# JuanTarrio/rebvo

Measured on NVIDIA H100. Metric: frames/sec @752x480 EuRoC replay (synthetic stand-in), detect+track+map; pose ATE vs reference in `parity`, higher is better.
Workload: dtype f32 scale space/detector + f64 tracker/EKF

## Files before the change

rebvo_b200/csrc/capi.cu:

```cuda
#include <math.h>
#include <stdlib.h>
#include <new>

#include "common.cuh"
#include "tracker.cuh"

int rb_detect_upload_pinv(rb_ctx *c);

static void box_plan_one(double sigma, int box_n, int *box_d, double *sigma_r) {
    const double wideal = sqrt(12 * sigma * sigma / box_n + 1);
    int wl = (int)wideal;
    const int tmp = wl / 2;
    if (tmp * 2 == wl) wl--;
    const int m = (int)round((3 * box_n + 4 * box_n * wl + box_n * wl * wl - 12 * sigma * sigma) / (4 + 4 * wl));
    int i = 0;
    for (; i < m && i < box_n; i++) box_d[i] = wl;
    for (; i < box_n; i++) box_d[i] = wl + 2;
    *sigma_r = sqrt((m * wl * wl + (box_n - m) * (wl + 2.0) * (wl + 2.0) - box_n) / 12.0);
}

static void plane_fit_pinv(double pinv[3][25]) {
    const int ws = 2;
    double Phi[25][3];
    int k = 0;
// ... 119 lines not shown
    kl.n_m0[i] = k.n_m0;
    kl.p_id[i] = k.p_id;
    kl.n_id[i] = k.n_id;
    kl.pack[2 * i] = make_float4(k.m_m[0], k.m_m[1], k.c_p[0], k.c_p[1]);
    kl.pack[2 * i + 1] = make_float4(k.u_m[0], k.u_m[1], k.n_m, 0.f);
}

__global__ void k_fill_int(int *p, int v, size_t n) {
    size_t i = (size_t)blockIdx.x * blockDim.x + threadIdx.x;
    if (i < n) p[i] = v;
}

extern "C" int rb_ctx_create(rb_ctx **out, int device, const rb_camera *cam, double sigma0, double ksigma,
                             int kl_capacity) {
    if (!out || !cam) return RB_ERR_ARG;
    *out = nullptr;
    int ndev = 0;
    if (cudaGetDeviceCount(&ndev) != cudaSuccess || ndev <= 0 || device >= ndev) return RB_ERR_NO_DEVICE;
    if (cam->w % 4 || cam->w < 32 || cam->h < 32 || kl_capacity < 1) return RB_ERR_ARG;
    rb_ctx *c = new (std::nothrow) rb_ctx;
    if (!c) return RB_ERR_ARG;
    memset(c, 0, sizeof(*c));
    c->mtx = new (std::nothrow) std::recursive_mutex;
    if (!c->mtx) {
        delete c;
        return RB_ERR_ARG;
    }
    c->device = device;
    c->cam = *cam;
    c->w = cam->w;
    c->h = cam->h;
    c->N = cam->w * cam->h;
    c->ppx = cam->ppx;
    c->ppy = cam->ppy;
    c->zfm = (double)((cam->zfx + cam->zfy) / 2);
    c->sigma0 = sigma0;
    c->ksigma = ksigma;
    c->kcap = kl_capacity;
    {
        const char *ds = getenv("REBVO_B200_DOG_SUB");
        c->dog_sub = ds ? atoi(ds) : 0;
        if (c->dog_sub < 0) c->dog_sub = 0;
        const char *pd = getenv("REBVO_B200_PDL");
        c->pdl = !(pd && atoi(pd) == 0);
        const char *mp = getenv("REBVO_B200_MIN_PERSIST");
        c->min_persist = !(mp && atoi(mp) == 0);
        const char *mc = getenv("REBVO_B200_MIN_CLUSTER");
        c->min_cluster = !(mc && atoi(mc) == 0);
        const char *rs = getenv("REBVO_B200_ROWSCAN");
        c->rowscan_mode = rs ? atoi(rs) : 2;
        c->mu_xchg = !(getenv("REBVO_B200_MU_XCHG") && atoi(getenv("REBVO_B200_MU_XCHG")) == 0);
        c->row_ns = getenv("REBVO_B200_ROW_NS") ? atoi(getenv("REBVO_B200_ROW_NS")) : 0;
        c->colscan_mode = getenv("REBVO_B200_COLSCAN") ? atoi(getenv("REBVO_B200_COLSCAN")) : 0;
    }
    box_plan_one(sigma0, 3, c->plan.d[0], &c->plan.sigma_r[0]);
    box_plan_one(c->plan.sigma_r[0] * ksigma, 3, c->plan.d[1], &c->plan.sigma_r[1]);
    plane_fit_pinv(c->pinv);
    int r = RB_OK;
    auto fail = [&](int code) {
        *out = c;
        return code;
    };
#define CK(call)                                                                                  \
    do {                                                                                          \
        cudaError_t e__ = (call);                                                                 \
        if (e__ != cudaSuccess) {                                                                 \
            snprintf(c->err, sizeof(c->err), "%s:%d %s: %s", __FILE__, __LINE__, #call,           \
                     cudaGetErrorString(e__));                                                    \
            return fail(RB_ERR_CUDA);                                                             \
        }                                                                                         \
    } while (0)
    CK(cudaSetDevice(device));
    cudaDeviceProp prop;
    CK(cudaGetDeviceProperties(&prop, device));
    c->sm_count = prop.multiProcessorCount;
    rb_minimizer_cluster_setup(c);
    if ((r = rb_dog_device_setup(c))) return fail(r);
    {
        int lo = 0, hi = 0;
        cudaDeviceGetStreamPriorityRange(&lo, &hi);
        const char *pe = getenv("REBVO_B200_PRIO");
        CK(cudaStreamCreateWithPriority(&c->stream, cudaStreamNonBlocking, (pe && atoi(pe) == 0) ? lo : hi));
    }
    c->nseg = c->h * rb_div_up(c->w, 32);
    CK(cudaMalloc(&c->seg_cnt, sizeof(int) * c->nseg));
    CK(cudaMalloc(&c->cand, sizeof(float4) * (size_t)c->N));
    c->red_cap = 1024;
    CK(cudaMalloc(&c->red_part, sizeof(double) * 32 * c->red_cap));
    CK(cudaMalloc(&c->ticket, sizeof(unsigned int) * 16));
    CK(cudaMemset(c->ticket, 0, sizeof(unsigned int) * 16));
    CK(cudaMallocHost(&c->pinned, 1 << 16));
    CK(cudaMalloc(&c->dev_small, 1 << 16));
    CK(cudaMemset(c->dev_small, 0, 1 << 16));
    {
        const int mm_init[2] = {-1, 0x7f7fffff};
        CK(cudaMemcpy((char *)c->dev_small + RB_DS_REEST, mm_init, sizeof(mm_init), cudaMemcpyHostToDevice));
    }
    if ((r = rb_detect_upload_pinv(c))) return fail(r);
    if ((r = rb_dog_make_tables(c))) return fail(r);
#undef CK
    *out = c;
    return RB_OK;
}

extern "C" void rb_ctx_destroy(rb_ctx *c) {
    if (!c) return;
// ... 340 lines not shown
```

rebvo_b200/csrc/common.cuh:

```cuda
#pragma once
#include <cuda_runtime.h>
#include <stdint.h>
#include <stdio.h>
#include <string.h>

#include <mutex>

#include "../../include/rebvo_b200.h"

#define RB_RHO_MAX 20.0
#define RB_RHO_MIN 1e-3
#define RB_RHO_INIT 1.0
#define RB_MAX_IMG_VALUE 765

struct KLSoA {
    int *p_inx;
    float2 *m_m, *u_m, *c_p, *p_m, *p_m_0, *m_m0;
    float *n_m;
    double *rho, *s_rho, *rho0, *s_rho0, *n_m0;
    int *m_id, *m_id_f, *m_num, *p_id, *n_id;
    float4 *pack;
};

struct MapState {
    int kn;
    int total_cand;
    float max_dog, min_dog;
    float retuned;
    float thresh_used;
    int nmatch;
    int fwd_match;
    int reg_num;
    unsigned int frame_count;
    int do_map;
    double s_rho_q;
    double Kp, RKp;
};

struct DetChain {
    double tresh;
    int l_kl_num;
    int pad;
};

struct BoxPlan {
    int d[2][3];
    double sigma_r[2];
};

struct DogWS {
    int B;
    uint8_t *rgb;
    float *gray;
    float *S;
    float *I0;
    float *I;
    float *img0;
    float *dog;
    float *aux;
    void *tmaps;
    bool tma_ok;
    int tma_row_mask;
    bool tma_row_ok;
};

struct rb_ctx {
    std::recursive_mutex *mtx;
    int device;
    cudaStream_t stream;
    rb_camera cam;
    int w, h, N;
    float ppx, ppy;
    double zfm;
    double sigma0, ksigma;
    int kcap;
    BoxPlan plan;
    double pinv[3][25];
    int64_t launches;
    int sm_count;
    char err[256];
    int *seg_cnt;
    int nseg;
    float4 *cand;
    double *red_part;
    int red_cap;
    unsigned int *ticket;
    void *pinned;
    void *dev_small;
    float *boxtab;
    bool counters_preset;
    int dog_sub;
    bool pdl;
    bool min_persist;
    bool min_cluster;
    int min_cluster_kpc;
    size_t min_cluster_dyn;
    int min_cluster_g;
    int min_cluster_kpc_multi;
    size_t min_cluster_dyn_multi;
    int min_debug_abort;
    bool mu_xchg;
    bool min_early;
    int min_cluster_xchg;
    int row_ns;
    int colscan_mode;
    int rowscan_mode;
};
#define RB_DS_REEST 0
#define RB_DS_CHAIN 32768
#define RB_DS_ARGS 36864
#define RB_DS_TMA_FAIL 45056
#define RB_DS_QHISTO 49152

struct LMState {
    double Xeval[6];
    int res_in, res_out;
    double max_r;
    double match_thresh, s_rho_min, k_huber;
    unsigned int match_num_thresh, frame_count;
    int iter_max, init_type, init_iter;
    double Vel_in[3], W0_in[3];
    double X[6], Xnew[6], Xt[6], h[6];
    double JtJ[36], JtF[6], JtJn[36], JtFn[6];
    double F, Fnew, F0, Ft, F0t, u, v, ut, vt, gain;
    int eff_steps, eff_steps_t;
    int iR, iRN, iRt;
    int n_eval;
    double Vel[3], W0[3], RVel[9], RW0[9], W_X[36];
    double rel_error, rel_error_score, score;
    double last_score;
    int no_keylines, pad_;
};

struct TrackState {
    LMState lm;
    int *blk_has;
    double *blk_last_fi;
    double *partials;
    double *carry;
    int nblk;
    struct MinCtl *ctl;
    unsigned long long *ll;
    struct FmBest *fm_best;
    double *reg_r, *reg_s;
    unsigned char *reg_set;
};


struct rb_map {
    rb_ctx *c;
    DogWS ws;
    bool owns_ws;
    float *img0, *dog;
    int *mask;
    unsigned long long *field;
    KLSoA kl;
    MapState *st;
    double *res[3];
    unsigned char *carry_flag[3];
// ... 75 lines not shown
```

rebvo_b200/csrc/dog.cu:

```cuda
#include <stdlib.h>
#include <new>

#include "common.cuh"

#define BOX_TAB_W 8
#define BOX_TAB_N (BOX_TAB_W * BOX_TAB_W)
__device__ __forceinline__ float box_avg(const float *__restrict__ I, int x, int y, int w, int h, int d,
                                         int d2, const float *__restrict__ tab) {
    const bool left = x < d2 + 1, right = x >= w - d2;
    const bool top = y < d2 + 1, bottom = y >= h - d2;
    const int xr = right ? w - 1 : x + d2;
    const int yb = bottom ? h - 1 : y + d2;
    const int xl = left ? 0 : x - d2 - 1, yt = top ? 0 : y - d2 - 1;
    const float A = I[yb * w + xr], B = I[yb * w + xl], C = I[yt * w + xr], D = I[yt * w + xl];
    const float t1 = bottom ? C : B, t2 = bottom ? B : C;
    const bool h1 = bottom ? !top : !left, h2 = bottom ? !left : !top;
    float r = A;
    r = h1 ? r - t1 : r;
    r = h2 ? r - t2 : r;
    r = (!top && !left) ? r + D : r;
    const int cx = left ? x + d2 + 1 : (right ? w - x + d2 : d);
    const int cy = top ? y + d2 + 1 : (bottom ? h - y + d2 : d);
    return r * tab[(cy - d2 - 1) * BOX_TAB_W + (cx - d2 - 1)];
}
// ... 284 lines not shown
            for (int f = 0; f < 2; f++) {
                const int d = f ? d1 : d0, d2 = f ? d21 : d20;
                const bool top = y < d2 + 1, bottom = y >= h - d2;
                const int jb = ly + d < jbmax[f] ? ly + d : jbmax[f];
                int cyi = (top ? y + d2 + 1 : (bottom ? h - y + d2 : d)) - d2 - 1;
                cyi = cyi < 0 ? 0 : cyi;
                const float A = rr[f][jb * BT_BW], B = ll[f][jb * BT_BW], C = rr[f][ly * BT_BW], D = ll[f][ly * BT_BW];
                const float t1 = bottom ? C : B, t2 = bottom ? B : C;
                float r = A - t1;
                r = r - t2;
                r = r + D;
                v[f] = r * tc[f][cyi * BOX_TAB_W];
            }
            sm.o0[ly][lx] = v[0];
            sm.o1[ly][lx] = v[1] - v[0];
        }
    }
    asm volatile("fence.proxy.async.shared::cta;" ::: "memory");
    __syncthreads();
    if (tid == 0) {
        const unsigned int s0 = (unsigned int)__cvta_generic_to_shared(&sm.o0[0][0]);
        const unsigned int s1 = (unsigned int)__cvta_generic_to_shared(&sm.o1[0][0]);
        const int z = out_slot + b;
        asm volatile("cp.async.bulk.tensor.3d.global.shared::cta.bulk_group [%0, {%1, %2, %3}], [%4];" ::"l"(&tm_img0),
                     "r"(x0), "r"(y0), "r"(z), "r"(s0)
                     : "memory");
        asm volatile("cp.async.bulk.tensor.3d.global.shared::cta.bulk_group [%0, {%1, %2, %3}], [%4];" ::"l"(&tm_dog), "r"(x0),
                     "r"(y0), "r"(z), "r"(s1)
                     : "memory");
        asm volatile("cp.async.bulk.commit_group;" ::: "memory");
        asm volatile("cp.async.bulk.wait_group.read 0;" ::: "memory");
    }
}

typedef CUresult (*PFN_tmapEncodeTiled)(CUtensorMap *, CUtensorMapDataType, cuuint32_t, void *, const cuuint64_t *,
                                        const cuuint64_t *, const cuuint32_t *, const cuuint32_t *, CUtensorMapInterleave,
                                        CUtensorMapSwizzle, CUtensorMapL2promotion, CUtensorMapFloatOOBfill);
static bool make_tmap3(CUtensorMap *tm, float *base, int w, int h, int nimg, int bw, int bh, bool swizzle128 = false) {
    static PFN_tmapEncodeTiled enc = nullptr;
    if (!enc) {
        void *fn = nullptr;
        cudaDriverEntryPointQueryResult qr;
        if (cudaGetDriverEntryPoint("cuTensorMapEncodeTiled", &fn, cudaEnableDefault, &qr) != cudaSuccess || !fn) return false;
        enc = (PFN_tmapEncodeTiled)fn;
    }
    const cuuint64_t dims[3] = {(cuuint64_t)w, (cuuint64_t)h, (cuuint64_t)nimg};
    const cuuint64_t strides[2] = {(cuuint64_t)w * 4, (cuuint64_t)w * h * 4};
    const cuuint32_t box[3] = {(cuuint32_t)bw, (cuuint32_t)bh, 1};
    const cuuint32_t es[3] = {1, 1, 1};
    return enc(tm, CU_TENSOR_MAP_DATA_TYPE_FLOAT32, 3, base, dims, strides, box, es, CU_TENSOR_MAP_INTERLEAVE_NONE,
               swizzle128 ? CU_TENSOR_MAP_SWIZZLE_128B : CU_TENSOR_MAP_SWIZZLE_NONE, CU_TENSOR_MAP_L2_PROMOTION_L2_128B,
               CU_TENSOR_MAP_FLOAT_OOB_FILL_NONE) == CUDA_SUCCESS;
}
enum { TM_I_BLUR = 0, TM_IMG0, TM_DOG, TM_GRAY, TM_S, TM_I0_F0, TM_I0_F1, TM_I_F0, TM_I_F1, TM_COUNT };
int rb_dog_make_tmaps(rb_ctx *c, DogWS *ws) {
    ws->tma_ok = false;
    ws->tma_row_ok = false;
    const char *e = getenv("REBVO_B200_BLUR_TMA");
    const char *er = getenv("REBVO_B200_ROW_TMA");
    const bool want_blur = !(e && atoi(e) == 0), want_row = !(er && atoi(er) == 0);
    if (!want_blur && !want_row) return RB_OK;
    if ((c->w * 4) % 16) return RB_OK;
    CUtensorMap *t = new (std::nothrow) CUtensorMap[TM_COUNT];
    if (!t) return RB_OK;
    ws->tmaps = t;
    if (want_blur) {
        bool ok = make_tmap3(&t[TM_I_BLUR], ws->I, c->w, c->h, 2 * ws->B, BT_BW, BT_BH) &&
                  make_tmap3(&t[TM_IMG0], ws->img0, c->w, c->h, ws->B, BT_W, BT_H) &&
                  make_tmap3(&t[TM_DOG], ws->dog, c->w, c->h, ws->B, BT_W, BT_H);
        ok = ok && cudaFuncSetAttribute(k_blur_dog_tma, cudaFuncAttributeMaxDynamicSharedMemorySize, (int)sizeof(BlurTmaSmem) + 128) == cudaSuccess;
        if (!ok) cudaGetLastError();
        ws->tma_ok = ok;
    }
    if (want_row) {
        const int (*d)[3] = c->plan.d;
        bool ok = make_tmap3(&t[TM_GRAY], ws->gray, c->w, c->h, ws->B, 32, 32, true) &&
                  make_tmap3(&t[TM_S], ws->S, c->w, c->h, 2 * ws->B, 32, 32, true) &&
                  make_tmap3(&t[TM_I0_F0], ws->I0, c->w, c->h, ws->B, 32, 32 + d[0][0]) &&
                  make_tmap3(&t[TM_I0_F1], ws->I0, c->w, c->h, ws->B, 32, 32 + d[1][0]) &&
                  make_tmap3(&t[TM_I_F0], ws->I, c->w, c->h, 2 * ws->B, 32, 32 + d[0][1]) &&
                  make_tmap3(&t[TM_I_F1], ws->I, c->w, c->h, 2 * ws->B, 32, 32 + d[1][1]);
        if (!ok) cudaGetLastError();
        ws->tma_row_ok = ok;
        ws->tma_row_mask = er ? atoi(er) : 1;
    }
    return RB_OK;
}

__global__ void k_gradient(const float *__restrict__ img0, float *__restrict__ dx, float *__restrict__ dy,
                           int w, int h) {
    const int x = blockIdx.x * blockDim.x + threadIdx.x;
    const int y = blockIdx.y;
    if (x >= w) return;
    float gx = 0.f, gy = 0.f;
    if (x >= 1 && x < w - 1 && y >= 1 && y < h - 1) {
        gx = img0[y * w + x + 1] - img0[y * w + x - 1];
        gy = img0[(y + 1) * w + x] - img0[(y - 1) * w + x];
    }
    dx[y * w + x] = gx;
    dy[y * w + x] = gy;
}

int rb_dogws_alloc(rb_ctx *c, DogWS *ws, int B) {
    memset(ws, 0, sizeof(*ws));
    ws->B = B;
    const size_t N = c->N;
    RB_CUDA(cudaMalloc(&ws->rgb, (size_t)B * 3 * N));
    RB_CUDA(cudaMalloc(&ws->gray, (size_t)B * N * 4));
    RB_CUDA(cudaMalloc(&ws->S, (size_t)2 * B * N * 4));
    RB_CUDA(cudaMalloc(&ws->I0, (size_t)B * N * 4));
    RB_CUDA(cudaMalloc(&ws->I, (size_t)2 * B * N * 4));
    RB_CUDA(cudaMalloc(&ws->img0, (size_t)B * N * 4));
    RB_CUDA(cudaMalloc(&ws->dog, (size_t)B * N * 4));
    RB_CUDA(cudaMalloc(&ws->aux, (size_t)3 * N * 4));
    return rb_dog_make_tmaps(c, ws);
}

void rb_dogws_free(DogWS *ws) {
    cudaFree(ws->rgb);
    cudaFree(ws->gray);
    cudaFree(ws->S);
    cudaFree(ws->I0);
    cudaFree(ws->I);
    cudaFree(ws->img0);
    cudaFree(ws->dog);
    cudaFree(ws->aux);
    delete[] (CUtensorMap *)ws->tmaps;
    memset(ws, 0, sizeof(*ws));
}

int rb_dog_gray(rb_ctx *c, DogWS *ws, int nimg, const void *const *src_pp) {
    const size_t n4 = (size_t)nimg * c->N / 4;
    k_rgb2gray<<<(unsigned)((n4 + 255) / 256), 256, 0, c->stream>>>((const uint32_t *)ws->rgb,
                                                                   (const uint32_t *const *)src_pp,
                                                                   (float4 *)ws->gray, n4);
    RB_LAUNCH_CHECK();
    return RB_OK;
}

#define RING_NS 4
#define RING_WARPS 4
__device__ __forceinline__ void cp_async16(void *smem_dst, const void *gsrc, int src_bytes) {
    const unsigned int s = (unsigned int)__cvta_generic_to_shared(smem_dst);
    asm volatile("cp.async.cg.shared.global [%0], [%1], 16, %2;\n" ::"r"(s), "l"(gsrc), "r"(src_bytes));
}
__device__ __forceinline__ void cp_async_commit() { asm volatile("cp.async.commit_group;\n" ::); }
template <int N>
__device__ __forceinline__ void cp_async_wait() {
    asm volatile("cp.async.wait_group %0;\n" ::"n"(N));
}

template <bool AVG>
__global__ void __launch_bounds__(32 * RING_WARPS) k_rowscan_ring(const float *__restrict__ in, float *__restrict__ out,
                                                                  int w, int h, int nimg, int in_mod, int nper, int d_f0,
                                                                  int d_f1, const float *__restrict__ tab_f0,
                                                                  const float *__restrict__ tab_f1, int rmax) {
    extern __shared__ __align__(16) float smem_ring[];
    const int warp = threadIdx.x >> 5, lane = threadIdx.x & 31;
    const int gw = blockIdx.x * RING_WARPS + warp;
    const int bands = (h + 31) >> 5;
    const int img = gw / bands, band = gw - img * bands;
    if (img >= nimg) return;
    float *ring = smem_ring + (size_t)warp * (RING_NS * rmax * 32 + 32 * 33 + BOX_TAB_N);
    float(*tile)[33] = reinterpret_cast<float(*)[33]>(ring + RING_NS * rmax * 32);
    float *tab = ring + RING_NS * rmax * 32 + 32 * 33;
    const size_t N = (size_t)w * h;
    const float *__restrict__ I = in + (size_t)(img % in_mod) * N;
    float *__restrict__ O = out + (size_t)img * N;
    const bool f1 = (img / nper) != 0;
    const int d = AVG ? (f1 ? d_f1 : d_f0) : 1;
    const int d2 = AVG ? d / 2 : 0;
    const int R = AVG ? 32 + d : 32;
    const int yb0 = AVG ? band * 32 - d2 - 1 : band * 32;
    if (AVG) {
        const float *__restrict__ tg = f1 ? tab_f1 : tab_f0;
        tab[lane] = tg[lane];
        tab[lane + 32] = tg[lane + 32];
    }
    const int y0 = band * 32;
// ... 68 lines not shown
            for (int r = 0; r < 32; r++) {
                const float v = col[r * 32];
                tile[r][lane] = (y0 + r < h && x < w) ? v : 0.f;
            }
        }
        __syncwarp();
        issue_chunk(AVG ? t - 1 + RING_NS : t + RING_NS - 1);
        float *row = tile[lane];
#pragma unroll
        for (int cidx = 0; cidx < 32; cidx++) {
            carry = carry + row[cidx];
            row[cidx] = carry;
        }
        __syncwarp();
        if (x < w) {
#pragma unroll 8
            for (int r = 0; r < 32; r++)
                if (y0 + r < h) O[(size_t)(y0 + r) * w + x] = tile[r][lane];
        }
        __syncwarp();
    }
    cp_async_wait<0>();
}

__device__ __forceinline__ unsigned int rt_s32(const void *p) { return (unsigned int)__cvta_generic_to_shared(p); }
__device__ __forceinline__ void rt_load3(unsigned int dst, const CUtensorMap *tm, int x, int y, int z, unsigned int bar,
                                         unsigned int bytes) {
    asm volatile("mbarrier.arrive.expect_tx.shared::cta.b64 _, [%0], %1;" ::"r"(bar), "r"(bytes) : "memory");
    asm volatile("cp.async.bulk.tensor.3d.shared::cluster.global.mbarrier::complete_tx::bytes [%0], [%1, {%2, %3, %4}], [%5];"
                 ::"r"(dst), "l"(tm), "r"(x), "r"(y), "r"(z), "r"(bar)
                 : "memory");
}
__device__ __forceinline__ void rt_store3(const CUtensorMap *tm, int x, int y, int z, unsigned int src) {
    asm volatile("cp.async.bulk.tensor.3d.global.shared::cta.bulk_group [%0, {%1, %2, %3}], [%4];" ::"l"(tm), "r"(x), "r"(y),
                 "r"(z), "r"(src)
                 : "memory");
    asm volatile("cp.async.bulk.commit_group;" ::: "memory");
}
__device__ __forceinline__ bool rt_wait(unsigned int bar, unsigned int parity, int *fail) {
    unsigned int ok = 0;
    const long long t0 = clock64();
    while (true) {
        asm volatile("{\n\t.reg .pred p;\n\tmbarrier.try_wait.parity.shared::cta.b64 p, [%1], %2;\n\tselp.u32 %0, 1, 0, p;\n\t}"
                     : "=r"(ok) : "r"(bar), "r"(parity) : "memory");
        if (ok) return true;
        if (clock64() - t0 > (1ll << 28)) {
            *fail = 1;
            return false;
        }
    }
}
__device__ __forceinline__ float rt_scan_tile(unsigned int tile_s, int lane, float carry) {
    const unsigned int rowp = tile_s + (unsigned int)((lane * 128) ^ ((lane & 7) << 4));
#pragma unroll
    for (int k = 0; k < 8; k++) {
        const unsigned int a = rowp ^ (unsigned int)(k << 4);
        float4 v;
        asm volatile("ld.shared.v4.f32 {%0, %1, %2, %3}, [%4];" : "=f"(v.x), "=f"(v.y), "=f"(v.z), "=f"(v.w) : "r"(a) : "memory");
        carry = carry + v.x;
        v.x = carry;
        carry = carry + v.y;
        v.y = carry;
        carry = carry + v.z;
        v.z = carry;
        carry = carry + v.w;
        v.w = carry;
        asm volatile("st.shared.v4.f32 [%0], {%1, %2, %3, %4};" ::"r"(a), "f"(v.x), "f"(v.y), "f"(v.z), "f"(v.w) : "memory");
    }
    return carry;
}

template <int RT_NS>
__global__ void __launch_bounds__(32) k_rowscan_tma_plain(const __grid_constant__ CUtensorMap tm_in,
                                                          const __grid_constant__ CUtensorMap tm_out, int w, int h,
                                                          int zin0, int *fail) {
    extern __shared__ unsigned char rt_raw[];
    unsigned char *base = rt_raw + ((1024u - (rt_s32(rt_raw) & 1023u)) & 1023u);
    unsigned long long *full = reinterpret_cast<unsigned long long *>(base + RT_NS * 4096);
    const int lane = threadIdx.x;
    const int bands = (h + 31) >> 5;
    const int img = blockIdx.x / bands, band = blockIdx.x - img * bands;
    const int y0 = band * 32;
    const int nchunk = (w + 31) >> 5;
    const unsigned int ring_s = rt_s32(base), full_s = rt_s32(full);
    if (lane == 0) {
#pragma unroll
        for (int k = 0; k < RT_NS; k++) asm volatile("mbarrier.init.shared::cta.b64 [%0], 1;" ::"r"(full_s + 8 * k) : "memory");
        asm volatile("fence.mbarrier_init.release.cluster;" ::: "memory");
#pragma unroll
        for (int ci = 0; ci < RT_NS - 1; ci++)
            if (ci < nchunk) rt_load3(ring_s + ci * 4096, &tm_in, 32 * ci, y0, zin0 + img, full_s + 8 * ci, 4096);
    }
    __syncwarp();
    float carry = 0.f;
    for (int t = 0; t < nchunk; t++) {
        const int slot = t % RT_NS;
        if (!rt_wait(full_s + 8 * slot, (unsigned int)(t / RT_NS) & 1u, fail)) break;
        carry = rt_scan_tile(ring_s + slot * 4096, lane, carry);
        asm volatile("fence.proxy.async.shared::cta;" ::: "memory");
        __syncwarp();
        if (lane == 0) {
            rt_store3(&tm_out, 32 * t, y0, img, ring_s + slot * 4096);
            asm volatile("cp.async.bulk.wait_group.read 1;" ::: "memory");
            const int cn = t + RT_NS - 1;
            if (cn < nchunk)
                rt_load3(ring_s + (cn % RT_NS) * 4096, &tm_in, 32 * cn, y0, zin0 + img, full_s + 8 * (cn % RT_NS), 4096);
        }
    }
    if (lane == 0) asm volatile("cp.async.bulk.wait_group.read 0;" ::: "memory");
}

template <int RT_NS>
__global__ void __launch_bounds__(32) k_rowscan_tma_avg(const __grid_constant__ CUtensorMap tm_in0,
                                                        const __grid_constant__ CUtensorMap tm_in1,
                                                        const __grid_constant__ CUtensorMap tm_out, int w, int h,
                                                        int in_mod, int nper, int d_f0, int d_f1,
                                                        const float *__restrict__ tab_f0, const float *__restrict__ tab_f1,
                                                        int rmax, int *fail) {
    extern __shared__ unsigned char rt_raw[];
    unsigned char *base = rt_raw + ((1024u - (rt_s32(rt_raw) & 1023u)) & 1023u);
    unsigned char *otile = base;
    float *ring = reinterpret_cast<float *>(base + 2 * 4096);
    unsigned long long *full = reinterpret_cast<unsigned long long *>(base + 2 * 4096 + (size_t)RT_NS * rmax * 128);
    float *tab = reinterpret_cast<float *>(full + RT_NS);
    const int lane = threadIdx.x;
    const int bands = (h + 31) >> 5;
    const int img = blockIdx.x / bands, band = blockIdx.x - img * bands;
    const bool f1 = (img / nper) != 0;
    const int d = f1 ? d_f1 : d_f0, d2 = d / 2;
    const int y0 = band * 32, yb0 = y0 - d2 - 1;
    const int zin = img % in_mod;
    const CUtensorMap *tm = f1 ? &tm_in1 : &tm_in0;
    const unsigned int wbytes = (unsigned int)(32 + d) * 128u;
    const int ntile = (w + 31) >> 5, nchunk = (w + 16 + 31) >> 5;
    const unsigned int ring_s = rt_s32(ring), full_s = rt_s32(full), ot_s = rt_s32(otile);
    const unsigned int slot_bytes = (unsigned int)rmax * 128u;
    {
        const float *__restrict__ tg = f1 ? tab_f1 : tab_f0;
        tab[lane] = tg[lane];
        tab[lane + 32] = tg[lane + 32];
    }
    if (lane == 0) {
#pragma unroll
        for (int k = 0; k < RT_NS; k++) asm volatile("mbarrier.init.shared::cta.b64 [%0], 1;" ::"r"(full_s + 8 * k) : "memory");
        asm volatile("fence.mbarrier_init.release.cluster;" ::: "memory");
#pragma unroll
        for (int ci = 0; ci < RT_NS - 1; ci++)
            if (ci < nchunk) rt_load3(ring_s + ci * slot_bytes, tm, 32 * ci - 16, yb0, zin, full_s + 8 * ci, wbytes);
    }
    __syncwarp();
    const bool band_interior = (y0 >= d2 + 1) && (y0 + 31 < h - d2);
    unsigned int so[8];
#pragma unroll
    for (int j = 0; j < 8; j++) so[j] = (unsigned int)((((lane >> 2) ^ j) << 4) | ((lane & 3) << 2));
    float carry = 0.f;
    bool ok = rt_wait(full_s, 0u, fail);
    for (int t = 0; ok && t < ntile; t++) {
        if (lane == 0) {
            asm volatile("cp.async.bulk.wait_group.read 1;" ::: "memory");
            const int cn = t + RT_NS - 1;
            if (cn < nchunk)
                rt_load3(ring_s + (cn % RT_NS) * slot_bytes, tm, 32 * cn - 16, yb0, zin, full_s + 8 * (cn % RT_NS), wbytes);
        }
        if (t + 1 < nchunk && !rt_wait(full_s + 8 * ((t + 1) % RT_NS), (unsigned int)((t + 1) / RT_NS) & 1u, fail)) break;
        __syncwarp();
        unsigned char *ot = otile + (t & 1) * 4096;
        const int x = t * 32 + lane;
        if (band_interior && t * 32 >= d2 + 1 && t * 32 + 31 < w - d2) {
            const int xr = x + d2 + 16, xl = x - d2 - 1 + 16;
            const float *colr = ring + (size_t)((xr >> 5) % RT_NS) * rmax * 32 + (xr & 31);
            const float *coll = ring + (size_t)((xl >> 5) % RT_NS) * rmax * 32 + (xl & 31);
            const float *colr_b = colr + d * 32, *coll_b = coll + d * 32;
            const float a = tab[d2 * BOX_TAB_W + d2];
#pragma unroll
            for (int r = 0; r < 32; r++) {
                float v = colr_b[r * 32] - coll_b[r * 32];
                v = v - colr[r * 32];
                v = v + coll[r * 32];
                *reinterpret_cast<float *>(ot + r * 128 + so[r & 7]) = v * a;
            }
        } else {
            const int xr = (x + d2 < w - 1 ? x + d2 : w - 1) + 16, xl = x - d2 - 1 + 16;
            const bool left = x < d2 + 1, right = x >= w - d2;
            int cxi = (left ? x + d2 + 1 : (right ? w - x + d2 : d)) - d2 - 1;
            cxi = cxi < 0 ? 0 : cxi;
            const float *colr = ring + (size_t)((xr >> 5) % RT_NS) * rmax * 32 + (xr & 31);
            const float *coll = ring + (size_t)((xl >> 5) % RT_NS) * rmax * 32 + (xl & 31);
            const float *tcol = tab + cxi;
            const int jbmax = h - 1 - yb0;
#pragma unroll
            for (int r = 0; r < 32; r++) {
                const int y = y0 + r;
                const bool top = y < d2 + 1, bottom = y >= h - d2;
                const int jb = r + d < jbmax ? r + d : jbmax;
                int cyi = (top ? y + d2 + 1 : (bottom ? h - y + d2 : d)) - d2 - 1;
                cyi = cyi < 0 ? 0 : cyi;
                const float A = colr[jb * 32], B = coll[jb * 32], C = colr[r * 32], Dd = coll[r * 32];
                const float t1 = bottom ? C : B, t2 = bottom ? B : C;
                float v = A - t1;
                v = v - t2;
                v = v + Dd;
                *reinterpret_cast<float *>(ot + r * 128 + so[r & 7]) = v * tcol[cyi * BOX_TAB_W];
            }
        }
        __syncwarp();
        carry = rt_scan_tile(ot_s + (t & 1) * 4096, lane, carry);
        asm volatile("fence.proxy.async.shared::cta;" ::: "memory");
        __syncwarp();
        if (lane == 0) rt_store3(&tm_out, 32 * t, y0, img, ot_s + (t & 1) * 4096);
    }
    if (lane == 0) asm volatile("cp.async.bulk.wait_group.read 0;" ::: "memory");
}

static int rowscan_tma(rb_ctx *c, DogWS *ws, int stage, const float *in, int nimg, int in_mod, int nper) {
    const CUtensorMap *t = (const CUtensorMap *)ws->tmaps;
    const int bands = (c->h + 31) / 32;
    int *fail = (int *)((char *)c->dev_small + RB_DS_TMA_FAIL);
    const int ns_env = c->row_ns;
    if (stage < 0) {
        const int zin0 = (int)((in - ws->gray) / (ptrdiff_t)c->N);
        const int ns = ns_env ? ns_env : 4;
#define RT_PLAIN(NS) k_rowscan_tma_plain<NS><<<nimg * bands, 32, NS * 4096 + 64 + 1024, c->stream>>>(t[TM_GRAY], t[TM_S], c->w, c->h, zin0, fail)
        if (ns >= 8) RT_PLAIN(8);
        else if (ns >= 6) RT_PLAIN(6);
        else RT_PLAIN(4);
#undef RT_PLAIN
    } else {
        const int d0 = c->plan.d[0][stage], d1 = c->plan.d[1][stage];
        const int rmax = 32 + (d0 > d1 ? d0 : d1);
        const int ns = ns_env ? ns_env : 4;
#define RT_AVG(NS)                                                                                                              \
    k_rowscan_tma_avg<NS><<<nimg * bands, 32, 2 * 4096 + (size_t)NS * rmax * 128 + 64 + BOX_TAB_N * 4 + 1024, c->stream>>>(     \
        t[stage == 0 ? TM_I0_F0 : TM_I_F0], t[stage == 0 ? TM_I0_F1 : TM_I_F1], t[TM_S], c->w, c->h, in_mod, nper, d0, d1,       \
        c->boxtab + (0 * 3 + stage) * BOX_TAB_N, c->boxtab + (1 * 3 + stage) * BOX_TAB_N, rmax, fail)
        if (ns >= 6) RT_AVG(6);
        else if (ns >= 5) RT_AVG(5);
        else if (ns == 3) RT_AVG(3);
        else RT_AVG(4);
#undef RT_AVG
    }
    RB_LAUNCH_CHECK();
    return RB_OK;
}

int rb_dog_device_setup(rb_ctx *c) {
    RB_CUDA(cudaFuncSetAttribute(k_rowscan_tma_avg<6>, cudaFuncAttributeMaxDynamicSharedMemorySize, 64 * 1024));
    RB_CUDA(cudaFuncSetAttribute(k_rowscan_ring<true>, cudaFuncAttributeMaxDynamicSharedMemorySize, 200 * 1024));
    RB_CUDA(cudaFuncSetAttribute(k_rowscan_ring<false>, cudaFuncAttributeMaxDynamicSharedMemorySize, 200 * 1024));
    return RB_OK;
}

static int rowscan_ring(rb_ctx *c, int stage, const float *in, float *out, int nimg, int in_mod, int nper) {
    const int bands = (c->h + 31) / 32;
    const int blocks = rb_div_up(nimg * bands, RING_WARPS);
    const int dmax = stage >= 0 ? (c->plan.d[0][stage] > c->plan.d[1][stage] ? c->plan.d[0][stage] : c->plan.d[1][stage]) : 0;
    const int rmax = 32 + dmax;
    const size_t smem = (size_t)RING_WARPS * (RING_NS * rmax * 32 + 32 * 33 + BOX_TAB_N) * sizeof(float);
    if (stage >= 0) {
        k_rowscan_ring<true><<<blocks, 32 * RING_WARPS, smem, c->stream>>>(
            in, out, c->w, c->h, nimg, in_mod, nper, c->plan.d[0][stage], c->plan.d[1][stage],
            c->boxtab + (0 * 3 + stage) * BOX_TAB_N, c->boxtab + (1 * 3 + stage) * BOX_TAB_N, rmax);
    } else {
        k_rowscan_ring<false><<<blocks, 32 * RING_WARPS, smem, c->stream>>>(in, out, c->w, c->h, nimg, in_mod, nper, 1, 1,
                                                                          nullptr, nullptr, rmax);
    }
    RB_LAUNCH_CHECK();
    return RB_OK;
}

static int rowscan(rb_ctx *c, DogWS *ws, int stage, const float *in, float *out, int nimg, int in_mod, int nper) {
    if (ws->tma_row_ok && out == ws->S && stage <= 1 && (ws->tma_row_mask == 1 || ws->tma_row_mask == (stage < 0 ? 2 : 3)) &&
        (stage < 0 ? (in >= ws->gray && in < ws->gray + (size_t)ws->B * c->N) : in == (stage == 0 ? ws->I0 : ws->I)))
        return rowscan_tma(c, ws, stage, in, nimg, in_mod, nper);
    if (c->rowscan_mode == 2) return rowscan_ring(c, stage, in, out, nimg, in_mod, nper);
    const int bands = (c->h + 31) / 32;
    const int warps = nimg * bands;
    const int blocks = rb_div_up(warps, 4);
    if (stage >= 0)
        k_rowscan<true><<<blocks, 128, 0, c->stream>>>(in, out, c->w, c->h, nimg, in_mod, nper, c->plan.d[0][stage],
                                                       c->plan.d[1][stage], c->boxtab + (0 * 3 + stage) * BOX_TAB_N,
                                                       c->boxtab + (1 * 3 + stage) * BOX_TAB_N);
    else
        k_rowscan<false><<<blocks, 128, 0, c->stream>>>(in, out, c->w, c->h, nimg, in_mod, nper, 1, 1, nullptr, nullptr);
    RB_LAUNCH_CHECK();
    return RB_OK;
}

static int blur_dog(rb_ctx *c, DogWS *ws, int nimg, float *img1_opt, int out_slot = 0) {
    if (ws->tma_ok && !img1_opt) {
        const CUtensorMap *t = (const CUtensorMap *)ws->tmaps;
        dim3 tg(rb_div_up(c->w, BT_W), rb_div_up(c->h, BT_H), nimg);
        k_blur_dog_tma<<<tg, BT_THREADS, sizeof(BlurTmaSmem) + 128, c->stream>>>(
            t[TM_I_BLUR], t[TM_IMG0], t[TM_DOG], c->w, c->h, nimg, out_slot, c->plan.d[0][2], c->plan.d[1][2],
            c->boxtab + (0 * 3 + 2) * BOX_TAB_N, c->boxtab + (1 * 3 + 2) * BOX_TAB_N, (int *)((char *)c->dev_small + RB_DS_TMA_FAIL));
        RB_LAUNCH_CHECK();
        return RB_OK;
    }
    dim3 grid(rb_div_up(c->w, 256), rb_div_up(c->h, BLUR_RY), nimg);
    const size_t off = (size_t)out_slot * c->N;
    k_blur_dog<<<grid, 256, 0, c->stream>>>(ws->I, ws->img0 + off, ws->dog + off, img1_opt, c->w, c->h, nimg,
                                            c->plan.d[0][2],
                                            c->plan.d[1][2], c->boxtab + (0 * 3 + 2) * BOX_TAB_N,
                                            c->boxtab + (1 * 3 + 2) * BOX_TAB_N);
    RB_LAUNCH_CHECK();
    return RB_OK;
}

int rb_dog_make_tables(rb_ctx *c) {
    float host[6 * BOX_TAB_N];
    for (int f = 0; f < 2; f++)
        for (int i = 0; i < 3; i++) {
            const int d = c->plan.d[f][i], d2 = d / 2;
            if (d2 + 1 > BOX_TAB_W) {
                snprintf(c->err, sizeof(c->err), "box width %d too large for this build", d);
                return RB_ERR_ARG;
            }
            float *t = host + (f * 3 + i) * BOX_TAB_N;
            for (int k = 0; k < BOX_TAB_N; k++) t[k] = 0.f;
            for (int cy = d2 + 1; cy <= d; cy++)
                for (int cx = d2 + 1; cx <= d; cx++) {
                    const float area = (float)(cx * cy);
                    t[(cy - d2 - 1) * BOX_TAB_W + (cx - d2 - 1)] = (float)(1.0 / (double)area);
                }
        }
    RB_CUDA(cudaMalloc(&c->boxtab, sizeof(host)));
    RB_CUDA(cudaMemcpy(c->boxtab, host, sizeof(host), cudaMemcpyHostToDevice));
    return RB_OK;
}

static int colscan(rb_ctx *c, const float *in, float *out, int nimg) {
    const int mode = c->colscan_mode;
#define COL_PIPE(VW, U)                                                                                                \
    k_colscan_pipe<VW, U><<<rb_div_up(nimg * (c->w / VW), 64), 64, 0, c->stream>>>(                                      \
        (const ColVec<VW>::T *)in, (ColVec<VW>::T *)out, c->w / VW, c->h, nimg)
    if (mode != 1) COL_PIPE(4, 16);
    else {
        const int w4 = c->w / 4;
        const int threads = nimg * w4;
        k_colscan<<<rb_div_up(threads, 64), 64, 0, c->stream>>>((const float4 *)in, (float4 *)out, w4, c->h, nimg);
    }
#undef COL_PIPE
    RB_LAUNCH_CHECK();
    return RB_OK;
}

int rb_dog_build_range(rb_ctx *c, DogWS *ws, int f0, int m) {
    if (f0 < 0 || m < 1 || f0 + m > ws->B) return RB_ERR_ARG;
    int r;
    const size_t N = c->N;
    if ((r = rowscan(c, ws, -1, ws->gray + f0 * N, ws->S, m, m, m))) return r;
    if ((r = colscan(c, ws->S, ws->I0, m))) return r;
    if ((r = rowscan(c, ws, 0, ws->I0, ws->S, 2 * m, m, m))) return r;
    if ((r = colscan(c, ws->S, ws->I, 2 * m))) return r;
    if ((r = rowscan(c, ws, 1, ws->I, ws->S, 2 * m, 2 * m, m))) return r;
    if ((r = colscan(c, ws->S, ws->I, 2 * m))) return r;
    return blur_dog(c, ws, m, nullptr, f0);
}

int rb_dog_build_batch(rb_ctx *c, DogWS *ws, int nimg) {
    if (nimg < 1 || nimg > ws->B) return RB_ERR_ARG;
    int r;
    const int sub = c->dog_sub > 0 ? c->dog_sub : nimg;
    for (int s = 0; s < nimg; s += sub)
        if ((r = rb_dog_build_range(c, ws, s, nimg - s < sub ? nimg - s : sub))) return r;
    return RB_OK;
}

int rb_dog_aux_planes(rb_ctx *c, DogWS *ws, int img) {
    if (ws->B != 1 || img != 0) return RB_ERR_ARG;
    int r = blur_dog(c, ws, 1, ws->aux);
    if (r) return r;
    dim3 grid(rb_div_up(c->w, 256), c->h, 1);
    k_gradient<<<grid, 256, 0, c->stream>>>(ws->img0, ws->aux + c->N, ws->aux + 2 * (size_t)c->N, c->w,
                                            c->h);
    RB_LAUNCH_CHECK();
    return RB_OK;
}

int rb_dog_single_pass(rb_ctx *c, DogWS *ws, int pass_id, int nimg, double *bytes) {
    const double N = (double)c->N;
    switch (pass_id) {
        case 0:
            *bytes = 8.0 * N * nimg;
            return rowscan(c, ws, -1, ws->gray, ws->S, nimg, nimg, nimg);
        case 1:
            *bytes = 8.0 * N * 2 * nimg;
            return rowscan(c, ws, 1, ws->I, ws->S, 2 * nimg, 2 * nimg, nimg);
        case 2:
            *bytes = 8.0 * N * 2 * nimg;
            return colscan(c, ws->S, ws->I, 2 * nimg);
        case 3:
            *bytes = 16.0 * N * nimg;
            return blur_dog(c, ws, nimg, nullptr);
        case 4:
            *bytes = 7.0 * N * nimg;
            return rb_dog_gray(c, ws, nimg);
        default:
            return RB_ERR_ARG;
    }
}
```

Measured before the change: 7290.

## Fuse column prefix scan into TMA row-scan kernels via decoupled look-back

Row-scan TMA kernels now also do the column integral-image scan in the same pass. Bands take work in order through an atomic ticket and pass per-column carries to the band below through sequence-tagged global slots with spin polling. This removes the three separate colscan launches and their global read/write round trips from the DoG build. It adds inter-block spin waits (with a timeout fallback), a global sync counter reset per launch, new tensor maps and extra memory, plus batched loads/stores in the tile scans.

```diff
diff --git a/rebvo_b200/csrc/capi.cu b/rebvo_b200/csrc/capi.cu
--- a/rebvo_b200/csrc/capi.cu
+++ b/rebvo_b200/csrc/capi.cu
@@ -195,6 +195,7 @@
         c->mu_xchg = !(getenv("REBVO_B200_MU_XCHG") && atoi(getenv("REBVO_B200_MU_XCHG")) == 0);
         c->row_ns = getenv("REBVO_B200_ROW_NS") ? atoi(getenv("REBVO_B200_ROW_NS")) : 0;
         c->colscan_mode = getenv("REBVO_B200_COLSCAN") ? atoi(getenv("REBVO_B200_COLSCAN")) : 0;
+        c->col_fused = !(getenv("REBVO_B200_COL_FUSED") && atoi(getenv("REBVO_B200_COL_FUSED")) == 0);
     }
     box_plan_one(sigma0, 3, c->plan.d[0], &c->plan.sigma_r[0]);
     box_plan_one(c->plan.sigma_r[0] * ksigma, 3, c->plan.d[1], &c->plan.sigma_r[1]);
diff --git a/rebvo_b200/csrc/common.cuh b/rebvo_b200/csrc/common.cuh
--- a/rebvo_b200/csrc/common.cuh
+++ b/rebvo_b200/csrc/common.cuh
@@ -62,6 +62,9 @@
     bool tma_ok;
     int tma_row_mask;
     bool tma_row_ok;
+    bool col_fused;
+    unsigned int *col_sync;
+    unsigned long long *col_slots;
 };
 
 struct rb_ctx {
@@ -105,6 +108,7 @@
     int row_ns;
     int colscan_mode;
     int rowscan_mode;
+    bool col_fused;
 };
 #define RB_DS_REEST 0
 #define RB_DS_CHAIN 32768
diff --git a/rebvo_b200/csrc/dog.cu b/rebvo_b200/csrc/dog.cu
--- a/rebvo_b200/csrc/dog.cu
+++ b/rebvo_b200/csrc/dog.cu
@@ -360,7 +360,8 @@
                swizzle128 ? CU_TENSOR_MAP_SWIZZLE_128B : CU_TENSOR_MAP_SWIZZLE_NONE, CU_TENSOR_MAP_L2_PROMOTION_L2_128B,
                CU_TENSOR_MAP_FLOAT_OOB_FILL_NONE) == CUDA_SUCCESS;
 }
-enum { TM_I_BLUR = 0, TM_IMG0, TM_DOG, TM_GRAY, TM_S, TM_I0_F0, TM_I0_F1, TM_I_F0, TM_I_F1, TM_COUNT };
+enum { TM_I_BLUR = 0, TM_IMG0, TM_DOG, TM_GRAY, TM_S, TM_I0_F0, TM_I0_F1, TM_I_F0, TM_I_F1, TM_I0_SW, TM_S_F0, TM_S_F1, TM_I_SW,
+       TM_COUNT };
 int rb_dog_make_tmaps(rb_ctx *c, DogWS *ws) {
     ws->tma_ok = false;
     ws->tma_row_ok = false;
@@ -392,6 +393,24 @@
         ws->tma_row_ok = ok;
         ws->tma_row_mask = er ? atoi(er) : 1;
     }
+    if (ws->tma_row_ok && ws->tma_row_mask == 1 && c->col_fused && c->rowscan_mode == 2 && c->colscan_mode == 0) {
+        const int (*d)[3] = c->plan.d;
+        bool ok = make_tmap3(&t[TM_I0_SW], ws->I0, c->w, c->h, ws->B, 32, 32, true) &&
+                  make_tmap3(&t[TM_S_F0], ws->S, c->w, c->h, 2 * ws->B, 32, 32 + d[0][1]) &&
+                  make_tmap3(&t[TM_S_F1], ws->S, c->w, c->h, 2 * ws->B, 32, 32 + d[1][1]) &&
+                  make_tmap3(&t[TM_I_SW], ws->I, c->w, c->h, 2 * ws->B, 32, 32, true);
+        if (!ok) {
+            cudaGetLastError();
+            return RB_OK;
+        }
+        const size_t nslot = (size_t)2 * ws->B * ((c->h + 31) / 32) * ((c->w + 31) / 32) * 32;
+        void *p = nullptr;
+        RB_CUDA(cudaMalloc(&p, 256 + nslot * 8));
+        RB_CUDA(cudaMemset(p, 0, 256 + nslot * 8));
+        ws->col_sync = (unsigned int *)p;
+        ws->col_slots = (unsigned long long *)((char *)p + 256);
+        ws->col_fused = true;
+    }
     return RB_OK;
 }
 
@@ -433,6 +452,7 @@
     cudaFree(ws->img0);
     cudaFree(ws->dog);
     cudaFree(ws->aux);
+    cudaFree(ws->col_sync);
     delete[] (CUtensorMap *)ws->tmaps;
     memset(ws, 0, sizeof(*ws));
 }
@@ -607,34 +627,97 @@
 }
 __device__ __forceinline__ float rt_scan_tile(unsigned int tile_s, int lane, float carry) {
     const unsigned int rowp = tile_s + (unsigned int)((lane * 128) ^ ((lane & 7) << 4));
+    float4 v[8];
 #pragma unroll
     for (int k = 0; k < 8; k++) {
         const unsigned int a = rowp ^ (unsigned int)(k << 4);
-        float4 v;
-        asm volatile("ld.shared.v4.f32 {%0, %1, %2, %3}, [%4];" : "=f"(v.x), "=f"(v.y), "=f"(v.z), "=f"(v.w) : "r"(a) : "memory");
-        carry = carry + v.x;
-        v.x = carry;
-        carry = carry + v.y;
-        v.y = carry;
-        carry = carry + v.z;
-        v.z = carry;
-        carry = carry + v.w;
-        v.w = carry;
-        asm volatile("st.shared.v4.f32 [%0], {%1, %2, %3, %4};" ::"r"(a), "f"(v.x), "f"(v.y), "f"(v.z), "f"(v.w) : "memory");
+        asm volatile("ld.shared.v4.f32 {%0, %1, %2, %3}, [%4];" : "=f"(v[k].x), "=f"(v[k].y), "=f"(v[k].z), "=f"(v[k].w) : "r"(a) : "memory");
+    }
+#pragma unroll
+    for (int k = 0; k < 8; k++) {
+        carry = carry + v[k].x;
+        v[k].x = carry;
+        carry = carry + v[k].y;
+        v[k].y = carry;
+        carry = carry + v[k].z;
+        v[k].z = carry;
+        carry = carry + v[k].w;
+        v[k].w = carry;
+    }
+#pragma unroll
+    for (int k = 0; k < 8; k++) {
+        const unsigned int a = rowp ^ (unsigned int)(k << 4);
+        asm volatile("st.shared.v4.f32 [%0], {%1, %2, %3, %4};" ::"r"(a), "f"(v[k].x), "f"(v[k].y), "f"(v[k].z), "f"(v[k].w) : "memory");
     }
     return carry;
 }
 
-template <int RT_NS>
+#define CF_SPIN_LIMIT (1ll << 28)
+__device__ __forceinline__ void cf_begin(unsigned int *sync, int bands, int &img, int &band, unsigned int &gen) {
+    unsigned int tk = 0, g = 0;
+    if (threadIdx.x == 0) {
+        g = *(volatile unsigned int *)&sync[0];
+        tk = atomicAdd(&sync[1], 1u);
+    }
+    tk = __shfl_sync(~0u, tk, 0);
+    gen = __shfl_sync(~0u, g, 0);
+    img = (int)(tk / (unsigned int)bands);
+    band = (int)tk - img * bands;
+}
+__device__ __forceinline__ void cf_end(unsigned int *sync, unsigned int gen) {
+    if (threadIdx.x == 0) {
+        __threadfence();
+        if (atomicAdd(&sync[2], 1u) == gridDim.x - 1) {
+            atomicExch(&sync[1], 0u);
+            atomicExch(&sync[2], 0u);
+            atomicExch(&sync[0], gen + 1u == 0xffffffffu ? 0u : gen + 1u);
+        }
+    }
+}
+__device__ __forceinline__ void cf_put(unsigned long long *s, unsigned int seq, float v) {
+    asm volatile("st.relaxed.gpu.global.u64 [%0], %1;" ::"l"(s), "l"(((unsigned long long)seq << 32) | __float_as_uint(v)) : "memory");
+}
+__device__ __forceinline__ bool cf_poll(const unsigned long long *s, unsigned int seq, float &v) {
+    unsigned long long x;
+    asm volatile("ld.relaxed.gpu.global.u64 %0, [%1];" : "=l"(x) : "l"(s) : "memory");
+    v = __uint_as_float((unsigned int)x);
+    return __all_sync(~0u, (unsigned int)(x >> 32) == seq);
+}
+__device__ __forceinline__ float cf_col_tile(unsigned char *tile, const unsigned int (&so)[8], float carry, bool first) {
+    float v[32];
+#pragma unroll
+    for (int r = 0; r < 32; r++) v[r] = *reinterpret_cast<const float *>(tile + r * 128 + so[r & 7]);
+#pragma unroll
+    for (int r = 0; r < 32; r++) {
+        if (r == 0 && first) {
+            carry = v[0];
+        } else {
+            carry = carry + v[r];
+            v[r] = carry;
+        }
+    }
+#pragma unroll
+    for (int r = 0; r < 32; r++) *reinterpret_cast<float *>(tile + r * 128 + so[r & 7]) = v[r];
+    return carry;
+}
+__device__ __forceinline__ void cf_offsets(int lane, unsigned int (&so)[8]) {
+#pragma unroll
+    for (int j = 0; j < 8; j++) so[j] = (unsigned int)((((lane >> 2) ^ j) << 4) | ((lane & 3) << 2));
+}
+
+template <int RT_NS, bool COL>
 __global__ void __launch_bounds__(32) k_rowscan_tma_plain(const __grid_constant__ CUtensorMap tm_in,
                                                           const __grid_constant__ CUtensorMap tm_out, int w, int h,
-                                                          int zin0, int *fail) {
+                                                          int zin0, int *fail, unsigned long long *cslots,
+                                                          unsigned int *csync) {
     extern __shared__ unsigned char rt_raw[];
     unsigned char *base = rt_raw + ((1024u - (rt_s32(rt_raw) & 1023u)) & 1023u);
     unsigned long long *full = reinterpret_cast<unsigned long long *>(base + RT_NS * 4096);
     const int lane = threadIdx.x;
     const int bands = (h + 31) >> 5;
-    const int img = blockIdx.x / bands, band = blockIdx.x - img * bands;
+    int img = blockIdx.x / bands, band = blockIdx.x - img * bands;
+    unsigned int gen = 0;
+    if (COL) cf_begin(csync, bands, img, band, gen);
     const int y0 = band * 32;
     const int nchunk = (w + 31) >> 5;
     const unsigned int ring_s = rt_s32(base), full_s = rt_s32(full);
@@ -648,30 +731,75 @@
     }
     __syncwarp();
     float carry = 0.f;
-    for (int t = 0; t < nchunk; t++) {
-        const int slot = t % RT_NS;
-        if (!rt_wait(full_s + 8 * slot, (unsigned int)(t / RT_NS) & 1u, fail)) break;
-        carry = rt_scan_tile(ring_s + slot * 4096, lane, carry);
-        asm volatile("fence.proxy.async.shared::cta;" ::: "memory");
-        __syncwarp();
-        if (lane == 0) {
-            rt_store3(&tm_out, 32 * t, y0, img, ring_s + slot * 4096);
-            asm volatile("cp.async.bulk.wait_group.read 1;" ::: "memory");
-            const int cn = t + RT_NS - 1;
-            if (cn < nchunk)
-                rt_load3(ring_s + (cn % RT_NS) * 4096, &tm_in, 32 * cn, y0, zin0 + img, full_s + 8 * (cn % RT_NS), 4096);
+    auto store_refill = [&](int t, int slot) {
+        rt_store3(&tm_out, 32 * t, y0, img, ring_s + slot * 4096);
+        asm volatile("cp.async.bulk.wait_group.read 1;" ::: "memory");
+        const int cn = t + RT_NS - 1;
+        if (cn < nchunk)
+            rt_load3(ring_s + (cn % RT_NS) * 4096, &tm_in, 32 * cn, y0, zin0 + img, full_s + 8 * (cn % RT_NS), 4096);
+    };
+    if (!COL) {
+        for (int t = 0; t < nchunk; t++) {
+            const int slot = t % RT_NS;
+            if (!rt_wait(full_s + 8 * slot, (unsigned int)(t / RT_NS) & 1u, fail)) break;
+            carry = rt_scan_tile(ring_s + slot * 4096, lane, carry);
+            asm volatile("fence.proxy.async.shared::cta;" ::: "memory");
+            __syncwarp();
+            if (lane == 0) store_refill(t, slot);
+        }
+    } else {
+        const unsigned int seq = gen + 1u;
+        unsigned long long *mine = cslots + (((size_t)img * bands + band) * nchunk) * 32 + lane;
+        const unsigned long long *above = mine - (size_t)nchunk * 32;
+        unsigned int so[8];
+        cf_offsets(lane, so);
+        bool ok = true, look = band > 0;
+        int rs = 0;
+        long long t0 = clock64();
+        for (int t = 0; t < nchunk;) {
+            float cin = 0.f;
+            bool go = rs > t && (!look || cf_poll(above + t * 32, seq, cin));
+            if (!go && rs > t && __any_sync(~0u, clock64() - t0 > CF_SPIN_LIMIT)) {
+                if (lane == 0) *fail = 1;
+                look = false;
+                go = true;
+            }
+            if (go) {
+                const int slot = t % RT_NS;
+                const float cout = ok ? cf_col_tile(base + slot * 4096, so, cin, band == 0) : cin;
+                if (band + 1 < bands) cf_put(mine + t * 32, seq, cout);
+                if (ok) {
+                    asm volatile("fence.proxy.async.shared::cta;" ::: "memory");
+                    __syncwarp();
+                    if (lane == 0) store_refill(t, slot);
+                }
+                t++;
+                t0 = clock64();
+            } else if (rs < nchunk && rs <= t + RT_NS - 2) {
+                if (ok) {
+                    const int slot = rs % RT_NS;
+                    if (__all_sync(~0u, rt_wait(full_s + 8 * slot, (unsigned int)(rs / RT_NS) & 1u, fail))) {
+                        carry = rt_scan_tile(ring_s + slot * 4096, lane, carry);
+                        __syncwarp();
+                    } else {
+                        ok = false;
+                    }
+                }
+                rs++;
+            }
         }
     }
     if (lane == 0) asm volatile("cp.async.bulk.wait_group.read 0;" ::: "memory");
-}
-
-template <int RT_NS>
+    if (COL) cf_end(csync, gen);
+}
+
+template <int RT_NS, bool COL>
 __global__ void __launch_bounds__(32) k_rowscan_tma_avg(const __grid_constant__ CUtensorMap tm_in0,
                                                         const __grid_constant__ CUtensorMap tm_in1,
                                                         const __grid_constant__ CUtensorMap tm_out, int w, int h,
                                                         int in_mod, int nper, int d_f0, int d_f1,
                                                         const float *__restrict__ tab_f0, const float *__restrict__ tab_f1,
-                                                        int rmax, int *fail) {
+                                                        int rmax, int *fail, unsigned long long *cslots, unsigned int *csync) {
     extern __shared__ unsigned char rt_raw[];
     unsigned char *base = rt_raw + ((1024u - (rt_s32(rt_raw) & 1023u)) & 1023u);
     unsigned char *otile = base;
@@ -680,7 +808,9 @@
     float *tab = reinterpret_cast<float *>(full + RT_NS);
     const int lane = threadIdx.x;
     const int bands = (h + 31) >> 5;
-    const int img = blockIdx.x / bands, band = blockIdx.x - img * bands;
+    int img = blockIdx.x / bands, band = blockIdx.x - img * bands;
+    unsigned int gen = 0;
+    if (COL) cf_begin(csync, bands, img, band, gen);
     const bool f1 = (img / nper) != 0;
     const int d = f1 ? d_f1 : d_f0, d2 = d / 2;
     const int y0 = band * 32, yb0 = y0 - d2 - 1;
@@ -706,18 +836,15 @@
     __syncwarp();
     const bool band_interior = (y0 >= d2 + 1) && (y0 + 31 < h - d2);
     unsigned int so[8];
-#pragma unroll
-    for (int j = 0; j < 8; j++) so[j] = (unsigned int)((((lane >> 2) ^ j) << 4) | ((lane & 3) << 2));
+    cf_offsets(lane, so);
     float carry = 0.f;
-    bool ok = rt_wait(full_s, 0u, fail);
-    for (int t = 0; ok && t < ntile; t++) {
+    auto row_stage = [&](int t) -> bool {
         if (lane == 0) {
-            asm volatile("cp.async.bulk.wait_group.read 1;" ::: "memory");
             const int cn = t + RT_NS - 1;
             if (cn < nchunk)
                 rt_load3(ring_s + (cn % RT_NS) * slot_bytes, tm, 32 * cn - 16, yb0, zin, full_s + 8 * (cn % RT_NS), wbytes);
         }
-        if (t + 1 < nchunk && !rt_wait(full_s + 8 * ((t + 1) % RT_NS), (unsigned int)((t + 1) / RT_NS) & 1u, fail)) break;
+        if (t + 1 < nchunk && !rt_wait(full_s + 8 * ((t + 1) % RT_NS), (unsigned int)((t + 1) / RT_NS) & 1u, fail)) return false;
         __syncwarp();
         unsigned char *ot = otile + (t & 1) * 4096;
         const int x = t * 32 + lane;
@@ -727,13 +854,16 @@
             const float *coll = ring + (size_t)((xl >> 5) % RT_NS) * rmax * 32 + (xl & 31);
             const float *colr_b = colr + d * 32, *coll_b = coll + d * 32;
             const float a = tab[d2 * BOX_TAB_W + d2];
+            float o[32];
 #pragma unroll
             for (int r = 0; r < 32; r++) {
                 float v = colr_b[r * 32] - coll_b[r * 32];
                 v = v - colr[r * 32];
                 v = v + coll[r * 32];
-                *reinterpret_cast<float *>(ot + r * 128 + so[r & 7]) = v * a;
-            }
+                o[r] = v * a;
+            }
+#pragma unroll
+            for (int r = 0; r < 32; r++) *reinterpret_cast<float *>(ot + r * 128 + so[r & 7]) = o[r];
         } else {
             const int xr = (x + d2 < w - 1 ? x + d2 : w - 1) + 16, xl = x - d2 - 1 + 16;
             const bool left = x < d2 + 1, right = x >= w - d2;
@@ -743,6 +873,7 @@
             const float *coll = ring + (size_t)((xl >> 5) % RT_NS) * rmax * 32 + (xl & 31);
             const float *tcol = tab + cxi;
             const int jbmax = h - 1 - yb0;
+            float o[32];
 #pragma unroll
             for (int r = 0; r < 32; r++) {
                 const int y = y0 + r;
@@ -755,27 +886,80 @@
                 float v = A - t1;
                 v = v - t2;
                 v = v + Dd;
-                *reinterpret_cast<float *>(ot + r * 128 + so[r & 7]) = v * tcol[cyi * BOX_TAB_W];
-            }
+                o[r] = v * tcol[cyi * BOX_TAB_W];
+            }
+#pragma unroll
+            for (int r = 0; r < 32; r++) *reinterpret_cast<float *>(ot + r * 128 + so[r & 7]) = o[r];
         }
         __syncwarp();
         carry = rt_scan_tile(ot_s + (t & 1) * 4096, lane, carry);
+        __syncwarp();
+        return true;
+    };
+    auto store = [&](int t) {
         asm volatile("fence.proxy.async.shared::cta;" ::: "memory");
         __syncwarp();
         if (lane == 0) rt_store3(&tm_out, 32 * t, y0, img, ot_s + (t & 1) * 4096);
+    };
+    bool ok = rt_wait(full_s, 0u, fail);
+    if (!COL) {
+        for (int t = 0; ok && t < ntile; t++) {
+            if (lane == 0) asm volatile("cp.async.bulk.wait_group.read 1;" ::: "memory");
+            if (!row_stage(t)) break;
+            store(t);
+        }
+    } else {
+        ok = __all_sync(~0u, ok);
+        const unsigned int seq = gen + 1u;
+        unsigned long long *mine = cslots + (((size_t)img * bands + band) * ntile) * 32 + lane;
+        const unsigned long long *above = mine - (size_t)ntile * 32;
+        bool look = band > 0;
+        int rs = 0;
+        long long t0 = clock64();
+        for (int t = 0; t < ntile;) {
+            float cin = 0.f;
+            bool go = rs > t && (!look || cf_poll(above + t * 32, seq, cin));
+            if (!go && rs > t && __any_sync(~0u, clock64() - t0 > CF_SPIN_LIMIT)) {
+                if (lane == 0) *fail = 1;
+                look = false;
+                go = true;
+            }
+            if (go) {
+                const float cout = ok ? cf_col_tile(otile + (t & 1) * 4096, so, cin, band == 0) : cin;
+                if (band + 1 < bands) cf_put(mine + t * 32, seq, cout);
+                if (ok) store(t);
+                t++;
+                t0 = clock64();
+            } else if (rs < ntile && rs <= t + 1) {
+                if (ok) {
+                    if (lane == 0) {
+                        if (rs == t + 1) asm volatile("cp.async.bulk.wait_group.read 0;" ::: "memory");
+                        else asm volatile("cp.async.bulk.wait_group.read 1;" ::: "memory");
+                    }
+                    ok = __all_sync(~0u, row_stage(rs));
+                }
+                rs++;
+            }
+        }
     }
     if (lane == 0) asm volatile("cp.async.bulk.wait_group.read 0;" ::: "memory");
-}
-
+    if (COL) cf_end(csync, gen);
+}
+
+template <bool COL>
 static int rowscan_tma(rb_ctx *c, DogWS *ws, int stage, const float *in, int nimg, int in_mod, int nper) {
     const CUtensorMap *t = (const CUtensorMap *)ws->tmaps;
     const int bands = (c->h + 31) / 32;
     int *fail = (int *)((char *)c->dev_small + RB_DS_TMA_FAIL);
+    unsigned long long *cslots = COL ? ws->col_slots : nullptr;
+    unsigned int *csync = COL ? ws->col_sync : nullptr;
     const int ns_env = c->row_ns;
     if (stage < 0) {
         const int zin0 = (int)((in - ws->gray) / (ptrdiff_t)c->N);
         const int ns = ns_env ? ns_env : 4;
-#define RT_PLAIN(NS) k_rowscan_tma_plain<NS><<<nimg * bands, 32, NS * 4096 + 64 + 1024, c->stream>>>(t[TM_GRAY], t[TM_S], c->w, c->h, zin0, fail)
+        const CUtensorMap &out = t[COL ? TM_I0_SW : TM_S];
+#define RT_PLAIN(NS) \
+    k_rowscan_tma_plain<NS, COL><<<nimg * bands, 32, NS * 4096 + 64 + 1024, c->stream>>>(t[TM_GRAY], out, c->w, c->h, zin0, fail, cslots, csync)
         if (ns >= 8) RT_PLAIN(8);
         else if (ns >= 6) RT_PLAIN(6);
         else RT_PLAIN(4);
@@ -784,10 +968,12 @@
         const int d0 = c->plan.d[0][stage], d1 = c->plan.d[1][stage];
         const int rmax = 32 + (d0 > d1 ? d0 : d1);
         const int ns = ns_env ? ns_env : 4;
+        const int in0 = stage == 0 ? TM_I0_F0 : (COL ? TM_S_F0 : TM_I_F0), in1 = stage == 0 ? TM_I0_F1 : (COL ? TM_S_F1 : TM_I_F1);
+        const CUtensorMap &out = t[COL && stage == 1 ? TM_I_SW : TM_S];
 #define RT_AVG(NS)                                                                                                              \
-    k_rowscan_tma_avg<NS><<<nimg * bands, 32, 2 * 4096 + (size_t)NS * rmax * 128 + 64 + BOX_TAB_N * 4 + 1024, c->stream>>>(     \
-        t[stage == 0 ? TM_I0_F0 : TM_I_F0], t[stage == 0 ? TM_I0_F1 : TM_I_F1], t[TM_S], c->w, c->h, in_mod, nper, d0, d1,       \
-        c->boxtab + (0 * 3 + stage) * BOX_TAB_N, c->boxtab + (1 * 3 + stage) * BOX_TAB_N, rmax, fail)
+    k_rowscan_tma_avg<NS, COL><<<nimg * bands, 32, 2 * 4096 + (size_t)NS * rmax * 128 + 64 + BOX_TAB_N * 4 + 1024, c->stream>>>( \
+        t[in0], t[in1], out, c->w, c->h, in_mod, nper, d0, d1, c->boxtab + (0 * 3 + stage) * BOX_TAB_N,                           \
+        c->boxtab + (1 * 3 + stage) * BOX_TAB_N, rmax, fail, cslots, csync)
         if (ns >= 6) RT_AVG(6);
         else if (ns >= 5) RT_AVG(5);
         else if (ns == 3) RT_AVG(3);
@@ -799,7 +985,8 @@
 }
 
 int rb_dog_device_setup(rb_ctx *c) {
-    RB_CUDA(cudaFuncSetAttribute(k_rowscan_tma_avg<6>, cudaFuncAttributeMaxDynamicSharedMemorySize, 64 * 1024));
+    RB_CUDA(cudaFuncSetAttribute(k_rowscan_tma_avg<6, false>, cudaFuncAttributeMaxDynamicSharedMemorySize, 64 * 1024));
+    RB_CUDA(cudaFuncSetAttribute(k_rowscan_tma_avg<6, true>, cudaFuncAttributeMaxDynamicSharedMemorySize, 64 * 1024));
     RB_CUDA(cudaFuncSetAttribute(k_rowscan_ring<true>, cudaFuncAttributeMaxDynamicSharedMemorySize, 200 * 1024));
     RB_CUDA(cudaFuncSetAttribute(k_rowscan_ring<false>, cudaFuncAttributeMaxDynamicSharedMemorySize, 200 * 1024));
     return RB_OK;
@@ -826,7 +1013,7 @@
 static int rowscan(rb_ctx *c, DogWS *ws, int stage, const float *in, float *out, int nimg, int in_mod, int nper) {
     if (ws->tma_row_ok && out == ws->S && stage <= 1 && (ws->tma_row_mask == 1 || ws->tma_row_mask == (stage < 0 ? 2 : 3)) &&
         (stage < 0 ? (in >= ws->gray && in < ws->gray + (size_t)ws->B * c->N) : in == (stage == 0 ? ws->I0 : ws->I)))
-        return rowscan_tma(c, ws, stage, in, nimg, in_mod, nper);
+        return rowscan_tma<false>(c, ws, stage, in, nimg, in_mod, nper);
     if (c->rowscan_mode == 2) return rowscan_ring(c, stage, in, out, nimg, in_mod, nper);
     const int bands = (c->h + 31) / 32;
     const int warps = nimg * bands;
@@ -903,6 +1090,12 @@
     if (f0 < 0 || m < 1 || f0 + m > ws->B) return RB_ERR_ARG;
     int r;
     const size_t N = c->N;
+    if (ws->col_fused) {
+        if ((r = rowscan_tma<true>(c, ws, -1, ws->gray + f0 * N, m, m, m))) return r;
+        if ((r = rowscan_tma<true>(c, ws, 0, ws->I0, 2 * m, m, m))) return r;
+        if ((r = rowscan_tma<true>(c, ws, 1, ws->S, 2 * m, 2 * m, m))) return r;
+        return blur_dog(c, ws, m, nullptr, f0);
+    }
     if ((r = rowscan(c, ws, -1, ws->gray + f0 * N, ws->S, m, m, m))) return r;
     if ((r = colscan(c, ws->S, ws->I0, m))) return r;
     if ((r = rowscan(c, ws, 0, ws->I0, ws->S, 2 * m, m, m))) return r;
@@ -937,9 +1130,11 @@
     switch (pass_id) {
         case 0:
             *bytes = 8.0 * N * nimg;
+            if (ws->col_fused) return rowscan_tma<true>(c, ws, -1, ws->gray, nimg, nimg, nimg);
             return rowscan(c, ws, -1, ws->gray, ws->S, nimg, nimg, nimg);
         case 1:
             *bytes = 8.0 * N * 2 * nimg;
+            if (ws->col_fused) return rowscan_tma<true>(c, ws, 1, ws->S, 2 * nimg, 2 * nimg, nimg);
             return rowscan(c, ws, 1, ws->I, ws->S, 2 * nimg, 2 * nimg, nimg);
         case 2:
             *bytes = 8.0 * N * 2 * nimg;
```

After: 7390 (median of 6 runs). 1.01x the previous value.
